# lizardfs/lizardfs

Measured on AMD Instinct MI355X. Metric: GiB/s EC encode, ec(8,2) 64MiB stripes, higher is better.
Workload: dtype u8; 1 GPU; ec(8,2) encode, 1024x64MiB synthetic stripes/GPU, device-resident; k=8, m=2, stripe_bytes=67108864, stripes_per_gpu=1024, parallelism=independent stripe batches x1

## Files before the change

lizardfs_amd/csrc/crc_fold.h:

```cpp
#pragma once
#include <hip/hip_runtime.h>

#include <cstdint>

#include "crc_fold_consts.h"

__device__ __forceinline__ uint32_t crc_advance(uint32_t crc, uint32_t len2,
                                                const uint32_t *mats) {
	int i = 0;
	while (len2) {
		if (len2 & 1) {
			const uint32_t *M = mats + i * 32;
			uint32_t r = 0, v = crc;
#pragma unroll
			for (int j = 0; j < 32; ++j) {
				r ^= (v & 1) ? M[j] : 0u;
				v >>= 1;
			}
			crc = r;
		}
		len2 >>= 1;
		++i;
	}
	return crc;
}

template <uint64_t K>
__device__ __forceinline__ void clmul_acc(uint32_t a0, uint32_t a1,
                                          uint32_t &r0, uint32_t &r1,
                                          uint32_t &r2, uint32_t &r3) {
#pragma unroll
	for (int s = 0; s < 64; ++s) {
		if ((K >> s) & 1) {
			const int t = s & 31;
			uint32_t w0 = t ? (a0 << t) : a0;
			uint32_t w1 = t ? ((a1 << t) | (a0 >> (32 - t))) : a1;
			uint32_t w2 = t ? (a1 >> (32 - t)) : 0u;
			if (s < 32) {
				r0 ^= w0;
				r1 ^= w1;
				if (t) r2 ^= w2;
			} else {
				r1 ^= w0;
				r2 ^= w1;
				if (t) r3 ^= w2;
			}
		}
	}
}

template <uint64_t KL, uint64_t KH>
__device__ __forceinline__ void crc_fold16(uint32_t (&acc)[4], uint32_t d0,
                                           uint32_t d1, uint32_t d2,
                                           uint32_t d3) {
	uint32_t r0 = d0, r1 = d1, r2 = d2, r3 = d3;
	clmul_acc<KL>(acc[0], acc[1], r0, r1, r2, r3);
	clmul_acc<KH>(acc[2], acc[3], r0, r1, r2, r3);
	acc[0] = r0;
	acc[1] = r1;
	acc[2] = r2;
	acc[3] = r3;
}

template <int NACC>
__device__ __forceinline__ void crc_fold_step(uint32_t (&acc)[4],
                                              const uint4 &d) {
	static_assert(NACC == 1 || NACC == 2 || NACC == 4, "NACC in {1,2,4}");
	if constexpr (NACC == 1)
		crc_fold16<kCrcFoldKL1, kCrcFoldKH1>(acc, d.x, d.y, d.z, d.w);
	else if constexpr (NACC == 2)
		crc_fold16<kCrcFoldKL2, kCrcFoldKH2>(acc, d.x, d.y, d.z, d.w);
	else
		crc_fold16<kCrcFoldKL4, kCrcFoldKH4>(acc, d.x, d.y, d.z, d.w);
}

__device__ __forceinline__ uint32_t crc_reduce16(const uint32_t (&acc)[4],
                                                 const uint32_t *T0) {
	uint32_t s = 0;
#pragma unroll
	for (int w = 0; w < 4; ++w) {
		uint32_t v = acc[w];
#pragma unroll
		for (int b = 0; b < 4; ++b)
			s = (s >> 8) ^ T0[(s ^ (v >> (8 * b))) & 0xFFu];
	}
	return s;
}

template <bool AL16, bool NT = false>
__device__ __forceinline__ uint4 crc_ld16(const uint8_t *p) {
	if constexpr (AL16 && NT) {
		typedef unsigned int u32x4 __attribute__((ext_vector_type(4)));
		u32x4 v = __builtin_nontemporal_load((const u32x4 *)p);
		return make_uint4(v.x, v.y, v.z, v.w);
	} else if constexpr (AL16) {
		return *(const uint4 *)p;
	} else {
		const uint32_t *u = (const uint32_t *)p;
		return make_uint4(u[0], u[1], u[2], u[3]);
	}
}

template <int C, int NACC, bool AL16 = true, bool NT = false,
          bool PF = false, int BVO = 0>
__device__ uint32_t crc_block_wave_fold(const uint8_t *__restrict__ block,
                                        uint32_t block_len, uint32_t seed,
                                        const uint32_t *T0,
                                        const uint32_t *mats, int lane) {
	constexpr int BV = BVO ? BVO : (C >= 4 ? 4 : 8);
	static_assert(BV % NACC == 0, "burst must cover whole interleave groups");
	const uint32_t span = block_len / C;
	const uint32_t seg = span >> 6;
	const uint8_t *base = block + (uint32_t)lane * seg;
	uint32_t acc[C][NACC][4];
	uint4 w[C][BV];
	auto ldburst = [&](uint4 (&buf)[C][BV], uint32_t i) {
#pragma unroll
		for (int c = 0; c < C; ++c)
#pragma unroll
			for (int q = 0; q < BV; ++q)
				buf[c][q] = crc_ld16<AL16, NT>(base + c * span + i + q * 16);
	};
	auto foldburst = [&](uint4 (&buf)[C][BV]) {
#pragma unroll
		for (int q = 0; q < BV; ++q)
#pragma unroll
			for (int c = 0; c < C; ++c)
				crc_fold_step<NACC>(acc[c][q % NACC], buf[c][q]);
	};
	ldburst(w, 0);
#pragma unroll
	for (int c = 0; c < C; ++c) {
		const uint32_t raw0 =
		    ((c == 0 && lane == 0) ? seed : 0u) ^ 0xFFFFFFFFu;
#pragma unroll
		for (int a = 0; a < NACC; ++a) {
			acc[c][a][0] = w[c][a].x ^ (a == 0 ? raw0 : 0u);
			acc[c][a][1] = w[c][a].y;
			acc[c][a][2] = w[c][a].z;
			acc[c][a][3] = w[c][a].w;
		}
#pragma unroll
		for (int q = NACC; q < BV; ++q)
			crc_fold_step<NACC>(acc[c][q % NACC], w[c][q]);
	}
	if (PF) {
		uint4 w2[C][BV];
		uint32_t i = 16 * BV;
		if (i < seg) ldburst(w2, i);
		for (; i < seg; i += 2 * 16 * BV) {
			if (i + 16 * BV < seg) ldburst(w, i + 16 * BV);
			foldburst(w2);
			if (i + 16 * BV < seg) {
				if (i + 2 * 16 * BV < seg) ldburst(w2, i + 2 * 16 * BV);
				foldburst(w);
			}
		}
	} else {
		for (uint32_t i = 16 * BV; i < seg; i += 16 * BV) {
			ldburst(w, i);
			foldburst(w);
		}
	}
	uint32_t crc[C];
#pragma unroll
	for (int c = 0; c < C; ++c) {
		uint32_t r[4] = {acc[c][0][0], acc[c][0][1], acc[c][0][2],
		                 acc[c][0][3]};
#pragma unroll
		for (int a = 1; a < NACC; ++a)
			crc_fold16<kCrcFoldKL1, kCrcFoldKH1>(
			    r, acc[c][a][0], acc[c][a][1], acc[c][a][2], acc[c][a][3]);
		crc[c] = crc_reduce16(r, T0) ^ 0xFFFFFFFFu;
	}
	uint32_t len = seg;
#pragma unroll
	for (int s = 0; s < 6; ++s) {
		uint32_t olen = __shfl_down(len, 1 << s, 64);
#pragma unroll
		for (int c = 0; c < C; ++c) {
			uint32_t o = __shfl_down(crc[c], 1 << s, 64);
			crc[c] = crc_advance(crc[c], olen, mats) ^ o;
		}
		len += olen;
	}
	uint32_t a = crc[0];
#pragma unroll
	for (int c = 1; c < C; ++c) a = crc_advance(a, span, mats) ^ crc[c];
	return a;
}
```

lizardfs_amd/csrc/crc_fold_consts.h:

```cpp
#pragma once
#include <cstdint>
constexpr uint64_t kCrcFoldKL1 = 0x420840204040300ull;
constexpr uint64_t kCrcFoldKH1 = 0x181820000810001ull;
constexpr uint64_t kCrcFoldKL2 = 0xa800004400013000ull;
constexpr uint64_t kCrcFoldKH2 = 0x20040700010021ull;
constexpr uint64_t kCrcFoldKL4 = 0x418000200010010aull;
constexpr uint64_t kCrcFoldKH4 = 0x80002200021c80ull;
```

lizardfs_amd/csrc/ec_kernel.h:

```cpp
#pragma once
#include <hip/hip_runtime.h>
#include <cstdint>

constexpr int kThreads = 256;
constexpr uint32_t kChunkBytes = kThreads * 16;

__device__ __forceinline__ uint32_t lut16(uint32_t t0, uint32_t t1,
                                          uint32_t t2, uint32_t t3,
                                          uint32_t nib) {
	uint32_t s3 = nib & 0x07070707u;
	uint32_t lo = __builtin_amdgcn_perm(t1, t0, s3);
	uint32_t hi = __builtin_amdgcn_perm(t3, t2, s3);
	uint32_t msel = 0x03020100u | ((nib >> 1) & 0x04040404u);
	return __builtin_amdgcn_perm(hi, lo, msel);
}

__device__ __forceinline__ uint32_t gf_macc(uint32_t acc, uint32_t w,
                                            const uint4 &L, const uint4 &H) {
	uint32_t nl = w & 0x0f0f0f0fu;
	uint32_t nh = (w >> 4) & 0x0f0f0f0fu;
	return acc ^ lut16(L.x, L.y, L.z, L.w, nl) ^ lut16(H.x, H.y, H.z, H.w, nh);
}

template <int D, int CH>
__device__ __forceinline__ void gf_macc_all(uint4 (&acc)[D][CH], int c,
                                            const uint4 &w, const uint4 (&L)[D],
                                            const uint4 (&H)[D]) {
#pragma unroll
	for (int d = 0; d < D; ++d) {
		acc[d][c].x = gf_macc(acc[d][c].x, w.x, L[d], H[d]);
		acc[d][c].y = gf_macc(acc[d][c].y, w.y, L[d], H[d]);
		acc[d][c].z = gf_macc(acc[d][c].z, w.z, L[d], H[d]);
		acc[d][c].w = gf_macc(acc[d][c].w, w.w, L[d], H[d]);
	}
}

__device__ __forceinline__ uint32_t gf_macc_q(uint32_t acc, const uint4 &T,
                                              uint32_t f0, uint32_t f1,
                                              uint32_t f2, uint32_t f3) {
	uint32_t p0 = __builtin_amdgcn_perm(T.x, T.x, f0);
	uint32_t p1 = __builtin_amdgcn_perm(T.y, T.y, f1);
	uint32_t p2 = __builtin_amdgcn_perm(T.z, T.z, f2);
	uint32_t p3 = __builtin_amdgcn_perm(T.w, T.w, f3);
	return acc ^ p0 ^ p1 ^ p2 ^ p3;
}

template <int D, int CH>
__device__ __forceinline__ void gf_macc_all_q(uint4 (&acc)[D][CH], int c,
                                              const uint4 &w,
                                              const uint4 (&T)[D]) {
	constexpr uint32_t M = 0x03030303u;
	uint32_t f[4][4];
	const uint32_t ws[4] = {w.x, w.y, w.z, w.w};
#pragma unroll
	for (int q = 0; q < 4; ++q) {
		f[q][0] = ws[q] & M;
		f[q][1] = (ws[q] >> 2) & M;
		f[q][2] = (ws[q] >> 4) & M;
		f[q][3] = (ws[q] >> 6) & M;
	}
#pragma unroll
	for (int d = 0; d < D; ++d) {
		acc[d][c].x = gf_macc_q(acc[d][c].x, T[d], f[0][0], f[0][1], f[0][2], f[0][3]);
		acc[d][c].y = gf_macc_q(acc[d][c].y, T[d], f[1][0], f[1][1], f[1][2], f[1][3]);
		acc[d][c].z = gf_macc_q(acc[d][c].z, T[d], f[2][0], f[2][1], f[2][2], f[2][3]);
		acc[d][c].w = gf_macc_q(acc[d][c].w, T[d], f[3][0], f[3][1], f[3][2], f[3][3]);
	}
}

__device__ __forceinline__ uint32_t gf_macc_mr(uint32_t acc, const uint4 &T,
                                               uint32_t t6, uint32_t f0,
                                               uint32_t f1, uint32_t f2) {
	uint32_t p0 = __builtin_amdgcn_perm(T.y, T.x, f0);
	uint32_t p1 = __builtin_amdgcn_perm(T.w, T.z, f1);
	uint32_t p2 = __builtin_amdgcn_perm(t6, t6, f2);
	return acc ^ p0 ^ p1 ^ p2;
}

template <int D, int CH>
__device__ __forceinline__ void gf_macc_all_mr(uint4 (&acc)[D][CH], int c,
                                               const uint4 &w,
                                               const uint4 (&T)[D],
                                               const uint4 (&T6)[D]) {
	constexpr uint32_t M3 = 0x07070707u, M2 = 0x03030303u;
	uint32_t f[4][3];
	const uint32_t ws[4] = {w.x, w.y, w.z, w.w};
#pragma unroll
	for (int q = 0; q < 4; ++q) {
		f[q][0] = ws[q] & M3;
		f[q][1] = (ws[q] >> 3) & M3;
		f[q][2] = (ws[q] >> 6) & M2;
	}
#pragma unroll
	for (int d = 0; d < D; ++d) {
		acc[d][c].x = gf_macc_mr(acc[d][c].x, T[d], T6[d].x, f[0][0], f[0][1], f[0][2]);
		acc[d][c].y = gf_macc_mr(acc[d][c].y, T[d], T6[d].x, f[1][0], f[1][1], f[1][2]);
		acc[d][c].z = gf_macc_mr(acc[d][c].z, T[d], T6[d].x, f[2][0], f[2][1], f[2][2]);
		acc[d][c].w = gf_macc_mr(acc[d][c].w, T[d], T6[d].x, f[3][0], f[3][1], f[3][2]);
	}
}

__device__ __forceinline__ uint32_t xcd_remap(uint32_t b, uint32_t n) {
	uint32_t xcd = b & 7u, i = b >> 3;
	uint32_t q = n >> 3, r = n & 7u;
	return (xcd < r ? xcd * (q + 1) : r * (q + 1) + (xcd - r) * q) + i;
}

__device__ __forceinline__ uint4 ld_nt(const uint8_t *p) {
	typedef unsigned int u32x4 __attribute__((ext_vector_type(4)));
	u32x4 v = __builtin_nontemporal_load((const u32x4 *)p);
	return make_uint4(v.x, v.y, v.z, v.w);
}

template <int D, int CH, bool SWZ, bool NTST, bool NTLD = false,
          bool TPIPE = false, bool QL = false, bool MR = false>
__global__ __launch_bounds__(kThreads) void ec_encode_kernel(
    uint32_t part_len, int srcs, int dest_base,
    const uint8_t *__restrict__ gftbls_dev,
    const uint64_t *__restrict__ src_ptrs,
    const uint64_t *__restrict__ dst_ptrs,
    int dests_total, uint32_t tiles_per_part, uint32_t total_tiles) {
	static_assert(!(QL && TPIPE), "QL and TPIPE are mutually exclusive");
	static_assert(!(MR && (QL || TPIPE)), "MR excludes QL/TPIPE");
	constexpr uint32_t kTile = kChunkBytes * CH;
	extern __shared__ __attribute__((aligned(16))) uint8_t smem[];
	const uint32_t tid = threadIdx.x;

	{
		const int tw = QL ? 16 : 32;
		const uint8_t *src_tbl = gftbls_dev + (size_t)dest_base * srcs * tw;
		int nbytes = D * srcs * tw;
		for (int i = tid * 16; i < nbytes; i += kThreads * 16)
			*(uint4 *)(smem + i) = *(const uint4 *)(src_tbl + i);
	}
	__syncthreads();

	uint32_t b0 = SWZ ? xcd_remap(blockIdx.x, gridDim.x) : blockIdx.x;
	for (uint32_t tile = b0; tile < total_tiles; tile += gridDim.x) {
		uint32_t stripe = tile / tiles_per_part;
		uint32_t tin = tile - stripe * tiles_per_part;
		uint32_t base = tin * kTile + tid * 16u;
		const uint64_t *sp_tab = src_ptrs + (uint64_t)stripe * srcs;
		const uint64_t *dp_tab =
		    dst_ptrs + (uint64_t)stripe * dests_total + dest_base;

		uint4 acc[D][CH];
#pragma unroll
		for (int d = 0; d < D; ++d)
#pragma unroll
			for (int c = 0; c < CH; ++c)
				acc[d][c] = make_uint4(0, 0, 0, 0);

		if ((uint64_t)(tin + 1) * kTile <= part_len) {
			uint4 w[CH], wn[CH];
			uint4 L[TPIPE ? 2 : 1][D], H[QL ? 1 : (TPIPE ? 2 : 1)][D];
			auto tbl_read = [&](int j, uint4 (&Lb)[D], uint4 (&Hb)[D]) {
#pragma unroll
				for (int d = 0; d < D; ++d) {
					if (QL) {
						Lb[d] = *(const uint4 *)(smem +
						                         ((size_t)d * srcs + j) * 16);
					} else if (MR) {
						const uint8_t *tb =
						    smem + ((size_t)d * srcs + j) * 32;
						Lb[d] = *(const uint4 *)tb;
						Hb[d].x = *(const uint32_t *)(tb + 16);
					} else {
						const uint8_t *tb =
						    smem + ((size_t)d * srcs + j) * 32;
						Lb[d] = *(const uint4 *)tb;
						Hb[d] = *(const uint4 *)(tb + 16);
					}
				}
			};
			{
				const uint8_t *sp = (const uint8_t *)sp_tab[0];
#pragma unroll
				for (int c = 0; c < CH; ++c)
					w[c] = NTLD ? ld_nt(sp + (base + c * kChunkBytes))
					            : *(const uint4 *)(sp + (base + c * kChunkBytes));
			}
			auto step = [&](int j, uint4 (&Lc)[D], uint4 (&Hc)[D],
			                uint4 (&Ln)[D], uint4 (&Hn)[D]) {
				if (j + 1 < srcs) {
					const uint8_t *spn = (const uint8_t *)sp_tab[j + 1];
#pragma unroll
					for (int c = 0; c < CH; ++c)
						wn[c] = NTLD ? ld_nt(spn + (base + c * kChunkBytes))
						             : *(const uint4 *)(spn + (base + c * kChunkBytes));
					if (TPIPE) tbl_read(j + 1, Ln, Hn);
				}
				if (!TPIPE) tbl_read(j, Lc, Hc);
#pragma unroll
				for (int c = 0; c < CH; ++c) {
					if (QL)
						gf_macc_all_q<D, CH>(acc, c, w[c], Lc);
					else if (MR)
						gf_macc_all_mr<D, CH>(acc, c, w[c], Lc, Hc);
					else
						gf_macc_all<D, CH>(acc, c, w[c], Lc, Hc);
				}
#pragma unroll
				for (int c = 0; c < CH; ++c) w[c] = wn[c];
			};
			if (TPIPE) tbl_read(0, L[0], H[0]);
			int j = 0;
			for (; j + 1 < srcs; j += 2) {
				step(j, L[0], H[0], L[TPIPE ? 1 : 0], H[TPIPE ? 1 : 0]);
				step(j + 1, L[TPIPE ? 1 : 0], H[TPIPE ? 1 : 0], L[0], H[0]);
			}
			if (j < srcs) step(j, L[0], H[0], L[TPIPE ? 1 : 0], H[TPIPE ? 1 : 0]);
#pragma unroll
			for (int d = 0; d < D; ++d) {
				uint8_t *dp = (uint8_t *)dp_tab[d];
#pragma unroll
				for (int c = 0; c < CH; ++c) {
					uint4 *p = (uint4 *)(dp + (base + c * kChunkBytes));
					if (NTST) {
						typedef unsigned int u32x4
						    __attribute__((ext_vector_type(4)));
						u32x4 v = {acc[d][c].x, acc[d][c].y, acc[d][c].z,
						           acc[d][c].w};
						__builtin_nontemporal_store(v, (u32x4 *)p);
					} else {
						*p = acc[d][c];
					}
				}
			}
		} else {
// ... 47 lines not shown
```

lizardfs_amd/csrc/lizec_gpu.hip:

```cpp
#include <hip/hip_runtime.h>

#include <cstdint>
#include <cstdio>
#include <cstring>
#include <cstdlib>
#include <atomic>
#include <mutex>
#include <unordered_map>

#include "../../include/lizec.h"

#define LIZEC_CHECK(x)                                                   \
	do {                                                                 \
		hipError_t _e = (x);                                             \
		if (_e != hipSuccess) return LIZEC_EHIP;                         \
	} while (0)

#include "ec_kernel.h"
#include "ec_kernel_multi.h"
#include "ec_kernel_strided.h"
#include "ec_kernel_ragged.h"
#include "ec_kernel_view.h"
#include "crc_fold.h"
#include "crc_ranges.h"
// ... 52 lines not shown
		      T1[(u >> 16) & 0xff] ^ T0[u >> 24];                      \
	} while (0)
			LIZEC_CRC_WORD(w.x);
			LIZEC_CRC_WORD(w.y);
			LIZEC_CRC_WORD(w.z);
			LIZEC_CRC_WORD(w.w);
#undef LIZEC_CRC_WORD
		}
		crc ^= 0xFFFFFFFFu;

		uint32_t len = seg;
#pragma unroll
		for (int s = 0; s < 6; ++s) {
			uint32_t ocrc = __shfl_down(crc, 1 << s, 64);
			uint32_t olen = __shfl_down(len, 1 << s, 64);
			crc = crc_advance(crc, olen, mats) ^ ocrc;
			len += olen;
		}
		if (lane == 0) out[blk] = crc;
	}
}

template <int C, int BV, int SL = 16>
__device__ uint32_t crc_block_wave(const uint8_t *__restrict__ block,
                                   uint32_t block_len, uint32_t seed,
                                   const uint32_t *T, const uint32_t *mats,
                                   int lane) {
	const uint32_t span = block_len / C;
	const uint32_t seg = span >> 6;
	const uint8_t *base = block + (uint32_t)lane * seg;
	uint32_t crc[C];
#pragma unroll
	for (int c = 0; c < C; ++c)
		crc[c] = ((c == 0 && lane == 0) ? seed : 0u) ^ 0xFFFFFFFFu;
	for (uint32_t i = 0; i < seg; i += 16 * BV) {
		uint4 w[C][BV];
#pragma unroll
		for (int c = 0; c < C; ++c)
#pragma unroll
			for (int q = 0; q < BV; ++q)
				w[c][q] = *(const uint4 *)(base + c * span + i + q * 16);
#define LIZEC_CRC16(crc, v)                                              \
	do {                                                                 \
		uint32_t u0 = (crc) ^ (v).x, u1 = (v).y, u2 = (v).z, u3 = (v).w; \
		(crc) = T[15 * 256 + (u0 & 0xff)] ^                              \
		        T[14 * 256 + ((u0 >> 8) & 0xff)] ^                       \
		        T[13 * 256 + ((u0 >> 16) & 0xff)] ^                      \
		        T[12 * 256 + (u0 >> 24)] ^                               \
		        T[11 * 256 + (u1 & 0xff)] ^                              \
		        T[10 * 256 + ((u1 >> 8) & 0xff)] ^                       \
		        T[9 * 256 + ((u1 >> 16) & 0xff)] ^                       \
		        T[8 * 256 + (u1 >> 24)] ^                                \
		        T[7 * 256 + (u2 & 0xff)] ^                               \
		        T[6 * 256 + ((u2 >> 8) & 0xff)] ^                        \
		        T[5 * 256 + ((u2 >> 16) & 0xff)] ^                       \
		        T[4 * 256 + (u2 >> 24)] ^                                \
		        T[3 * 256 + (u3 & 0xff)] ^                               \
		        T[2 * 256 + ((u3 >> 8) & 0xff)] ^                        \
		        T[1 * 256 + ((u3 >> 16) & 0xff)] ^ T[u3 >> 24];          \
	} while (0)
#define LIZEC_CRC8(crc, lo, hi)                                          \
	do {                                                                 \
		uint32_t u0 = (crc) ^ (lo), u1 = (hi);                           \
		(crc) = T[7 * 256 + (u0 & 0xff)] ^                               \
		        T[6 * 256 + ((u0 >> 8) & 0xff)] ^                        \
		        T[5 * 256 + ((u0 >> 16) & 0xff)] ^                       \
		        T[4 * 256 + (u0 >> 24)] ^                                \
		        T[3 * 256 + (u1 & 0xff)] ^                               \
		        T[2 * 256 + ((u1 >> 8) & 0xff)] ^                        \
		        T[1 * 256 + ((u1 >> 16) & 0xff)] ^ T[u1 >> 24];          \
	} while (0)
#pragma unroll
		for (int q = 0; q < BV; ++q)
#pragma unroll
			for (int c = 0; c < C; ++c) {
				if (SL == 16) {
					LIZEC_CRC16(crc[c], w[c][q]);
				} else {
					LIZEC_CRC8(crc[c], w[c][q].x, w[c][q].y);
					LIZEC_CRC8(crc[c], w[c][q].z, w[c][q].w);
				}
			}
#undef LIZEC_CRC16
#undef LIZEC_CRC8
	}
#pragma unroll
	for (int c = 0; c < C; ++c) crc[c] ^= 0xFFFFFFFFu;

	uint32_t len = seg;
#pragma unroll
	for (int s = 0; s < 6; ++s) {
		uint32_t olen = __shfl_down(len, 1 << s, 64);
#pragma unroll
		for (int c = 0; c < C; ++c) {
			uint32_t o = __shfl_down(crc[c], 1 << s, 64);
			crc[c] = crc_advance(crc[c], olen, mats) ^ o;
		}
		len += olen;
	}
	uint32_t acc = crc[0];
#pragma unroll
	for (int c = 1; c < C; ++c)
		acc = crc_advance(acc, span, mats) ^ crc[c];
	return acc;
}

template <int C, int BV, int SL = 16>
__global__ __launch_bounds__(kThreads) void crc32_blocks_kernel_multi(
    const uint8_t *__restrict__ buf, uint32_t block_len, uint64_t nblocks,
    uint32_t seed, const uint32_t *__restrict__ crc_const,
    uint32_t *__restrict__ out) {
	__shared__ __attribute__((aligned(16))) uint32_t stabs[kCrcConstWords];
	for (int i = threadIdx.x; i < kCrcConstWords; i += kThreads)
		stabs[i] = crc_const[i];
	__syncthreads();
	const uint32_t *T = stabs;
	const uint32_t *mats = stabs + kCrcTabWords;
	const int wave = threadIdx.x >> 6;
	const int lane = threadIdx.x & 63;
	for (uint64_t blk = (uint64_t)blockIdx.x * 4 + wave; blk < nblocks;
	     blk += (uint64_t)gridDim.x * 4) {
		uint32_t crc = crc_block_wave<C, BV, SL>(buf + blk * block_len,
		                                         block_len, seed, T, mats,
		                                         lane);
		if (lane == 0) out[blk] = crc;
	}
}


constexpr int kCrcFoldLdsWords = 256 + kCrcMatCount * 32;

template <int C, int NACC, bool AL16 = true, bool NT = false,
          bool PF = false, int BVO = 0>
__global__ __launch_bounds__(kThreads) void crc32_blocks_kernel_fold(
    const uint8_t *__restrict__ buf, uint32_t block_len, uint64_t nblocks,
    uint32_t seed, const uint32_t *__restrict__ crc_const,
    uint32_t *__restrict__ out) {
	__shared__ __attribute__((aligned(16))) uint32_t stabs[kCrcFoldLdsWords];
	for (int i = threadIdx.x; i < 256; i += kThreads)
		stabs[i] = crc_const[i];
	for (int i = threadIdx.x; i < kCrcMatCount * 32; i += kThreads)
		stabs[256 + i] = crc_const[kCrcTabWords + i];
	__syncthreads();
	const int wave = threadIdx.x >> 6;
	const int lane = threadIdx.x & 63;
	for (uint64_t blk = (uint64_t)blockIdx.x * 4 + wave; blk < nblocks;
	     blk += (uint64_t)gridDim.x * 4) {
		uint32_t crc = crc_block_wave_fold<C, NACC, AL16, NT, PF, BVO>(
		    buf + blk * block_len, block_len, seed, stabs, stabs + 256, lane);
		if (lane == 0) out[blk] = crc;
	}
}

template <bool WRITE>
__global__ __launch_bounds__(kThreads) void scrub_chunks_kernel(
    const uint64_t *__restrict__ chunk_dptrs,
    const uint32_t *__restrict__ data_offs,
    const uint32_t *__restrict__ crc_offs,
    const uint32_t *__restrict__ block_counts, uint32_t nchunks,
    uint32_t max_blocks, uint32_t block_stride, uint32_t crc_stride,
    const uint32_t *__restrict__ crc_const, int32_t *__restrict__ status) {
	__shared__ __attribute__((aligned(16))) uint32_t stabs[kCrcFoldLdsWords];
	for (int i = threadIdx.x; i < 256; i += kThreads)
		stabs[i] = crc_const[i];
	for (int i = threadIdx.x; i < kCrcMatCount * 32; i += kThreads)
		stabs[256 + i] = crc_const[kCrcTabWords + i];
	__syncthreads();
	const uint32_t *T0 = stabs;
	const uint32_t *mats = stabs + 256;
	const int wave = threadIdx.x >> 6;
	const int lane = threadIdx.x & 63;
	const uint64_t total = (uint64_t)nchunks * max_blocks;
	for (uint64_t flat = (uint64_t)blockIdx.x * 4 + wave; flat < total;
	     flat += (uint64_t)gridDim.x * 4) {
		uint32_t c = (uint32_t)(flat / max_blocks);
		uint32_t b = (uint32_t)(flat - (uint64_t)c * max_blocks);
		if (b >= block_counts[c]) continue;
		const uint8_t *img = (const uint8_t *)chunk_dptrs[c];
		const uint8_t *blockp = img + data_offs[c] + b * block_stride;
		uint32_t crc =
		    (((uintptr_t)blockp & 15) == 0)
		        ? crc_block_wave_fold<1, 1, true>(blockp, 65536u, 0u, T0,
		                                          mats, lane)
		        : crc_block_wave_fold<1, 1, false>(blockp, 65536u, 0u, T0,
		                                           mats, lane);
		if (lane == 0) {
			uint8_t *p = (uint8_t *)img + crc_offs[c] + crc_stride * b;
			if (WRITE) {
				p[0] = (uint8_t)(crc >> 24);
				p[1] = (uint8_t)(crc >> 16);
				p[2] = (uint8_t)(crc >> 8);
				p[3] = (uint8_t)crc;
			} else {
				uint32_t stored = ((uint32_t)p[0] << 24) |
				                  ((uint32_t)p[1] << 16) |
				                  ((uint32_t)p[2] << 8) | p[3];
				if (stored != crc) atomicMin(&status[c], (int32_t)b);
			}
		}
	}
}


struct lizec_stream_ctx {
	uint8_t *d_gftbls = nullptr;
	uint64_t *d_ptrs = nullptr;
	size_t ptrs_cap = 0;
	uint8_t *h_staging = nullptr;
	size_t h_cap = 0;
	hipEvent_t uploaded = nullptr;
	bool ev_recorded = false;
	uint8_t *d_mtbls = nullptr;
	size_t mtbls_cap = 0;
	uint32_t *d_mindex = nullptr;
	size_t mindex_cap = 0;
	uint8_t *h_mstaging = nullptr;
	size_t h_mcap = 0;
	uint8_t *d_ragged = nullptr;
	uint8_t *h_ragged = nullptr;
	size_t ragged_cap = 0;
};

struct lizec_engine {
	int device;
	hipStream_t stream;
	uint32_t *d_crc_const;
	std::mutex mu;
	std::unordered_map<void *, lizec_stream_ctx> ctxs;
	std::atomic<int> crc_shape{-1};
};

static void ctx_free(lizec_stream_ctx &c) {
	(void)hipFree(c.d_gftbls);
	(void)hipFree(c.d_ptrs);
	(void)hipHostFree(c.h_staging);
	(void)hipFree(c.d_mtbls);
	(void)hipFree(c.d_mindex);
	(void)hipHostFree(c.h_mstaging);
	(void)hipFree(c.d_ragged);
	(void)hipHostFree(c.h_ragged);
	if (c.uploaded) (void)hipEventDestroy(c.uploaded);
	c = lizec_stream_ctx();
}

static int ctx_acquire(lizec_engine *e, hipStream_t s, size_t ptrs,
                       size_t staging, lizec_stream_ctx **out) {
	lizec_stream_ctx *cp;
	{
		std::lock_guard<std::mutex> lk(e->mu);
		cp = &e->ctxs[(void *)s];
	}
	lizec_stream_ctx &c = *cp;
	if (!c.uploaded) {
		if (hipEventCreateWithFlags(&c.uploaded, hipEventDisableTiming) !=
		    hipSuccess)
			return LIZEC_EHIP;
	}
	if (c.ev_recorded) {
		LIZEC_CHECK(hipEventSynchronize(c.uploaded));
		c.ev_recorded = false;
	}
	if (!c.d_gftbls)
		LIZEC_CHECK(hipMalloc(&c.d_gftbls, (size_t)kECTblBytes * 32 * 32));
	if (c.ptrs_cap < ptrs) {
		size_t cap = c.ptrs_cap ? c.ptrs_cap : (1 << 16);
		while (cap < ptrs) cap *= 2;
		(void)hipFree(c.d_ptrs);
		c.d_ptrs = nullptr;
		c.ptrs_cap = 0;
		LIZEC_CHECK(hipMalloc(&c.d_ptrs, cap * sizeof(uint64_t)));
		c.ptrs_cap = cap;
	}
	size_t want = staging + (size_t)kECTblBytes * 32 * 32;
	if (c.h_cap < want) {
		size_t cap = c.h_cap ? c.h_cap : (1 << 20);
		while (cap < want) cap *= 2;
		(void)hipHostFree(c.h_staging);
		c.h_staging = nullptr;
		c.h_cap = 0;
		LIZEC_CHECK(hipHostMalloc(&c.h_staging, cap));
		c.h_cap = cap;
	}
	*out = &c;
	return LIZEC_OK;
}

static int ctx_acquire_multi(lizec_engine *e, hipStream_t s, size_t ptrs,
                             size_t staging, size_t tbl_bytes, size_t stripes,
                             lizec_stream_ctx **out) {
	int r = ctx_acquire(e, s, ptrs, staging, out);
	if (r != LIZEC_OK) return r;
	lizec_stream_ctx &c = **out;
	if (c.mtbls_cap < tbl_bytes) {
		size_t cap = c.mtbls_cap ? c.mtbls_cap : (1 << 16);
		while (cap < tbl_bytes) cap *= 2;
		(void)hipFree(c.d_mtbls);
		c.d_mtbls = nullptr;
		c.mtbls_cap = 0;
		LIZEC_CHECK(hipMalloc(&c.d_mtbls, cap));
		c.mtbls_cap = cap;
	}
	if (c.mindex_cap < stripes) {
		size_t cap = c.mindex_cap ? c.mindex_cap : (1 << 14);
		while (cap < stripes) cap *= 2;
		(void)hipFree(c.d_mindex);
		c.d_mindex = nullptr;
		c.mindex_cap = 0;
		LIZEC_CHECK(hipMalloc(&c.d_mindex, cap * sizeof(uint32_t)));
		c.mindex_cap = cap;
	}
	size_t want = tbl_bytes + stripes * sizeof(uint32_t);
	if (c.h_mcap < want) {
		size_t cap = c.h_mcap ? c.h_mcap : (1 << 17);
		while (cap < want) cap *= 2;
		(void)hipHostFree(c.h_mstaging);
		c.h_mstaging = nullptr;
		c.h_mcap = 0;
		LIZEC_CHECK(hipHostMalloc(&c.h_mstaging, cap));
		c.h_mcap = cap;
	}
	return LIZEC_OK;
}

static int ctx_acquire_ragged(lizec_engine *e, hipStream_t s, size_t ptrs,
                              size_t staging, size_t bytes,
                              lizec_stream_ctx **out) {
	int r = ctx_acquire(e, s, ptrs, staging, out);
	if (r != LIZEC_OK) return r;
	lizec_stream_ctx &c = **out;
	if (c.ragged_cap < bytes) {
		size_t cap = c.ragged_cap ? c.ragged_cap : (1 << 17);
		while (cap < bytes) cap *= 2;
		(void)hipFree(c.d_ragged);
		(void)hipHostFree(c.h_ragged);
		c.d_ragged = c.h_ragged = nullptr;
		c.ragged_cap = 0;
		LIZEC_CHECK(hipMalloc(&c.d_ragged, cap));
		LIZEC_CHECK(hipHostMalloc(&c.h_ragged, cap));
// ... 706 lines not shown
	                           hipMemcpyHostToDevice, s));
	LIZEC_CHECK(hipMemcpyAsync(c->d_mindex, istage, (size_t)num_stripes * 4,
	                           hipMemcpyHostToDevice, s));
	LIZEC_CHECK(hipMemcpyAsync(d_src, pstage, (nsrc + ndst) * 8,
	                           hipMemcpyHostToDevice, s));
	LIZEC_CHECK(hipEventRecord(c->uploaded, s));
	c->ev_recorded = true;

	return run_batch_multi(part_len, srcs, dests, c->d_mtbls, c->d_mindex,
	                       d_src, d_dst, (uint32_t)num_stripes, s);
}

extern "C" int lizec_ec_plan_create_multi(lizec_engine *e, uint64_t part_len,
                                          int srcs, int dests,
                                          const uint8_t *gftbls, int ntables,
                                          const uint32_t *tbl_index,
                                          const uint64_t *src_dptrs,
                                          const uint64_t *dst_dptrs,
                                          int num_stripes, lizec_plan **out) {
	*out = nullptr;
	if (!e) return LIZEC_EINVAL;
	int r = check_multi_args(part_len, srcs, dests, gftbls, ntables,
	                         tbl_index, src_dptrs, dst_dptrs, num_stripes);
	if (r != LIZEC_OK) return r;
	LIZEC_CHECK(hipSetDevice(e->device));
	size_t nsrc = (size_t)num_stripes * srcs;
	size_t ndst = (size_t)num_stripes * dests;
	size_t ntbl = (size_t)ntables * srcs * dests;
	size_t tbl_bytes = ntbl * kECTblBytes;
	uint8_t *packed = (uint8_t *)malloc(tbl_bytes);
	if (!packed) return LIZEC_ENOMEM;
	for (size_t i = 0; i < ntbl; ++i)
		pack_mixed_radix(gftbls + i * 32, packed + i * kECTblBytes);
	lizec_plan *p = new lizec_plan();
	p->e = e;
	p->part_len = part_len;
	p->srcs = srcs;
	p->dests = dests;
	p->num_stripes = num_stripes;
	if (hipMalloc(&p->d_tbls, tbl_bytes) != hipSuccess ||
	    hipMalloc(&p->d_src, nsrc * 8) != hipSuccess ||
	    hipMalloc(&p->d_dst, ndst * 8) != hipSuccess ||
	    hipMalloc(&p->d_index, (size_t)num_stripes * 4) != hipSuccess) {
		free(packed);
		lizec_ec_plan_destroy(p);
		return LIZEC_ENOMEM;
	}
	bool ok = hipMemcpy(p->d_tbls, packed, tbl_bytes,
	                    hipMemcpyHostToDevice) == hipSuccess &&
	          hipMemcpy(p->d_index, tbl_index, (size_t)num_stripes * 4,
	                    hipMemcpyHostToDevice) == hipSuccess &&
	          hipMemcpy(p->d_src, src_dptrs, nsrc * 8,
	                    hipMemcpyHostToDevice) == hipSuccess &&
	          hipMemcpy(p->d_dst, dst_dptrs, ndst * 8,
	                    hipMemcpyHostToDevice) == hipSuccess;
	free(packed);
	if (!ok) {
		lizec_ec_plan_destroy(p);
		return LIZEC_EHIP;
	}
	*out = p;
	return LIZEC_OK;
}

extern "C" int lizec_ec_plan_create(lizec_engine *e, uint64_t part_len,
                                    int srcs, int dests,
                                    const uint8_t *gftbls,
                                    const uint64_t *src_dptrs,
                                    const uint64_t *dst_dptrs,
                                    int num_stripes, lizec_plan **out) {
	*out = nullptr;
	if (!e) return LIZEC_EINVAL;
	int r = check_batch_args(part_len, srcs, dests, num_stripes);
	if (r != LIZEC_OK) return r;
	size_t nsrc = (size_t)num_stripes * srcs;
	size_t ndst = (size_t)num_stripes * dests;
	r = check_part_addrs(src_dptrs, nsrc, dst_dptrs, ndst);
	if (r != LIZEC_OK) return r;
	LIZEC_CHECK(hipSetDevice(e->device));
	lizec_plan *p = new lizec_plan();
	p->e = e;
	p->part_len = part_len;
	p->srcs = srcs;
	p->dests = dests;
	p->num_stripes = num_stripes;
	if (hipMalloc(&p->d_tbls, (size_t)kECTblBytes * srcs * dests) != hipSuccess ||
	    hipMalloc(&p->d_src, nsrc * 8) != hipSuccess ||
	    hipMalloc(&p->d_dst, ndst * 8) != hipSuccess) {
		lizec_ec_plan_destroy(p);
		return LIZEC_ENOMEM;
	}
	uint8_t packed[kECTblBytes * 32 * 32];
	for (int i = 0; i < srcs * dests; ++i)
		pack_mixed_radix(gftbls + (size_t)i * 32, packed + (size_t)i * kECTblBytes);
	if (hipMemcpy(p->d_tbls, packed, (size_t)kECTblBytes * srcs * dests,
	              hipMemcpyHostToDevice) != hipSuccess ||
	    hipMemcpy(p->d_src, src_dptrs, nsrc * 8,
	              hipMemcpyHostToDevice) != hipSuccess ||
	    hipMemcpy(p->d_dst, dst_dptrs, ndst * 8,
	              hipMemcpyHostToDevice) != hipSuccess) {
		lizec_ec_plan_destroy(p);
		return LIZEC_EHIP;
	}
	*out = p;
	return LIZEC_OK;
}

extern "C" int lizec_ec_plan_run(lizec_plan *p, void *stream) {
	if (!p) return LIZEC_EINVAL;
	hipStream_t s = stream ? (hipStream_t)stream : p->e->stream;
	LIZEC_CHECK(hipSetDevice(p->e->device));
	if (p->d_index)
		return run_batch_multi(p->part_len, p->srcs, p->dests, p->d_tbls,
		                       p->d_index, p->d_src, p->d_dst,
		                       (uint32_t)p->num_stripes, s);
	return run_batch(p->part_len, p->srcs, p->dests, p->d_tbls, p->d_src,
	                 p->d_dst, (uint32_t)p->num_stripes, s);
}

extern "C" void lizec_ec_plan_destroy(lizec_plan *p) {
	if (!p) return;
	(void)hipFree(p->d_tbls);
	(void)hipFree(p->d_src);
	(void)hipFree(p->d_dst);
	(void)hipFree(p->d_index);
	delete p;
}

extern "C" int lizec_crc32_batch(lizec_engine *e, const void *dev_buf,
                                 uint32_t block_len, uint64_t nblocks,
                                 uint32_t seed, uint32_t *dev_crcs_out,
                                 void *stream) {
	if (!e || !dev_buf || !dev_crcs_out || nblocks < 1) return LIZEC_EINVAL;
	if (block_len == 0 || (block_len & 1023)) return LIZEC_EINVAL;
	if (block_len >= (2u << kCrcMatCount)) return LIZEC_EINVAL;
	if ((uintptr_t)dev_buf & 3) return LIZEC_EINVAL;
	hipStream_t s = stream ? (hipStream_t)stream : e->stream;
	LIZEC_CHECK(hipSetDevice(e->device));
	uint64_t groups = (nblocks + 3) / 4;
	uint32_t grid = (uint32_t)(groups < 131072 ? groups : 131072);
	const char *ch = getenv("LIZEC_CRC_CHAINS");
	const char *sl = getenv("LIZEC_CRC_SLICE");
	const char *im = getenv("LIZEC_CRC_IMPL");
	const char *fn = getenv("LIZEC_CRC_FOLD_NACC");
	const char *nt = getenv("LIZEC_CRC_NT");
	const char *pf = getenv("LIZEC_CRC_PF");
	int chains = ch ? atoi(ch) : 1;
	int slice = sl ? atoi(sl) : 8;
	bool fold = !(im && strcmp(im, "table") == 0);
	int nacc = fn ? atoi(fn) : 1;
	bool ntld = nt && atoi(nt) != 0;
	bool pfld = pf && atoi(pf) != 0;
	bool al16 = (((uintptr_t)dev_buf | block_len) & 15) == 0;
	if (!al16 && (!fold || block_len % (64 * 16 * 8) != 0)) {
		hipLaunchKernelGGL(HIP_KERNEL_NAME(crc32_blocks_kernel<false>),
		                   dim3(grid), dim3(kThreads), 0, s,
		                   (const uint8_t *)dev_buf, block_len, nblocks,
		                   seed, e->d_crc_const, dev_crcs_out);
		LIZEC_CHECK(hipGetLastError());
		return LIZEC_OK;
	}
	if (!al16 && !(chains == 2 && block_len % (2 * 64 * 16 * 8) == 0))
		chains = 1;
	if (fold && block_len % ((uint32_t)chains * 64 * 16 * 8) == 0 &&
	    (chains == 1 || chains == 2)) {
		const uint8_t *b = (const uint8_t *)dev_buf;
#define LIZEC_LAUNCH_FOLD(C, N, A, NT)                                       \
	hipLaunchKernelGGL(HIP_KERNEL_NAME(crc32_blocks_kernel_fold<C, N, A, NT>), \
	                   dim3(grid), dim3(kThreads), 0, s, b, block_len,       \
	                   nblocks, seed, e->d_crc_const, dev_crcs_out)
		if (!al16) {
			if (chains == 2) LIZEC_LAUNCH_FOLD(2, 2, false, false);
			else LIZEC_LAUNCH_FOLD(1, 1, false, false);
		} else if (chains == 2) {
			if (nacc == 1) LIZEC_LAUNCH_FOLD(2, 1, true, false);
			else LIZEC_LAUNCH_FOLD(2, 2, true, false);
		} else if (pfld) {
			const char *bv = getenv("LIZEC_CRC_BV");
			if (bv && atoi(bv) == 4)
				hipLaunchKernelGGL(HIP_KERNEL_NAME(crc32_blocks_kernel_fold<1, 1, true, false, true, 4>),
				                   dim3(grid), dim3(kThreads), 0, s, b,
				                   block_len, nblocks, seed, e->d_crc_const,
				                   dev_crcs_out);
			else
				hipLaunchKernelGGL(HIP_KERNEL_NAME(crc32_blocks_kernel_fold<1, 1, true, false, true>),
				                   dim3(grid), dim3(kThreads), 0, s, b,
				                   block_len, nblocks, seed, e->d_crc_const,
				                   dev_crcs_out);
		} else if (ntld) {
			if (nacc == 1) LIZEC_LAUNCH_FOLD(1, 1, true, true);
			else if (nacc == 4) LIZEC_LAUNCH_FOLD(1, 4, true, true);
			else LIZEC_LAUNCH_FOLD(1, 2, true, true);
		} else {
			const char *bv = getenv("LIZEC_CRC_BV");
			const char *at = getenv("LIZEC_CRC_AUTOTUNE");
			bool tune = !(at && atoi(at) == 0);
			if (bv && atoi(bv) == 4 && nacc == 1) {
				hipLaunchKernelGGL(HIP_KERNEL_NAME(crc32_blocks_kernel_fold<1, 1, true, false, false, 4>),
				                   dim3(grid), dim3(kThreads), 0, s, b,
				                   block_len, nblocks, seed, e->d_crc_const,
				                   dev_crcs_out);
			} else if (nacc == 4) {
				if (bv && atoi(bv) == 4)
					hipLaunchKernelGGL(HIP_KERNEL_NAME(crc32_blocks_kernel_fold<1, 4, true, false, false, 4>),
					                   dim3(grid), dim3(kThreads), 0, s, b,
					                   block_len, nblocks, seed,
					                   e->d_crc_const, dev_crcs_out);
				else
					LIZEC_LAUNCH_FOLD(1, 4, true, false);
			} else if (nacc == 2) {
				if (bv && atoi(bv) == 4)
					hipLaunchKernelGGL(HIP_KERNEL_NAME(crc32_blocks_kernel_fold<1, 2, true, false, false, 4>),
					                   dim3(grid), dim3(kThreads), 0, s, b,
					                   block_len, nblocks, seed,
					                   e->d_crc_const, dev_crcs_out);
				else
					LIZEC_LAUNCH_FOLD(1, 2, true, false);
			} else {
				int shape = e->crc_shape.load(std::memory_order_relaxed);
				if (shape < 0 && tune && nblocks >= 4096) {
					hipEvent_t ev[3];
					int made = 0;
					for (; made < 3; ++made)
						if (hipEventCreate(&ev[made]) != hipSuccess) break;
					if (made == 3) {
						(void)hipEventRecord(ev[0], s);
						LIZEC_LAUNCH_FOLD(1, 1, true, false);
						(void)hipEventRecord(ev[1], s);
						hipLaunchKernelGGL(HIP_KERNEL_NAME(crc32_blocks_kernel_fold<1, 1, true, false, true>),
						                   dim3(grid), dim3(kThreads), 0, s,
						                   b, block_len, nblocks, seed,
						                   e->d_crc_const, dev_crcs_out);
						(void)hipEventRecord(ev[2], s);
						if (hipEventSynchronize(ev[2]) == hipSuccess) {
							float t0 = 0.f, t1 = 0.f;
							(void)hipEventElapsedTime(&t0, ev[0], ev[1]);
							(void)hipEventElapsedTime(&t1, ev[1], ev[2]);
							shape = (t1 > 0.f && t1 < t0) ? 1 : 0;
							e->crc_shape.store(shape,
							                   std::memory_order_relaxed);
						}
					} else {
						LIZEC_LAUNCH_FOLD(1, 1, true, false);
					}
					for (int i = 0; i < made; ++i)
						(void)hipEventDestroy(ev[i]);
					LIZEC_CHECK(hipGetLastError());
					return LIZEC_OK;
				}
				if (shape == 1)
					hipLaunchKernelGGL(HIP_KERNEL_NAME(crc32_blocks_kernel_fold<1, 1, true, false, true>),
					                   dim3(grid), dim3(kThreads), 0, s, b,
					                   block_len, nblocks, seed,
					                   e->d_crc_const, dev_crcs_out);
				else
					LIZEC_LAUNCH_FOLD(1, 1, true, false);
			}
		}
#undef LIZEC_LAUNCH_FOLD
		LIZEC_CHECK(hipGetLastError());
		return LIZEC_OK;
	}
	if (block_len % 32768 == 0 && chains >= 4)
		hipLaunchKernelGGL(HIP_KERNEL_NAME(crc32_blocks_kernel_multi<4, 8>),
		                   dim3(grid), dim3(kThreads), 0, s,
		                   (const uint8_t *)dev_buf, block_len, nblocks,
		                   seed, e->d_crc_const, dev_crcs_out);
	else if (block_len % 16384 == 0 && slice == 8)
		hipLaunchKernelGGL(HIP_KERNEL_NAME(crc32_blocks_kernel_multi<2, 8, 8>),
		                   dim3(grid), dim3(kThreads), 0, s,
		                   (const uint8_t *)dev_buf, block_len, nblocks,
		                   seed, e->d_crc_const, dev_crcs_out);
	else if (block_len % 16384 == 0)
		hipLaunchKernelGGL(HIP_KERNEL_NAME(crc32_blocks_kernel_multi<2, 8>),
		                   dim3(grid), dim3(kThreads), 0, s,
		                   (const uint8_t *)dev_buf, block_len, nblocks,
		                   seed, e->d_crc_const, dev_crcs_out);
	else
		hipLaunchKernelGGL(HIP_KERNEL_NAME(crc32_blocks_kernel<true>),
		                   dim3(grid), dim3(kThreads), 0, s,
		                   (const uint8_t *)dev_buf, block_len, nblocks,
		                   seed, e->d_crc_const, dev_crcs_out);
	LIZEC_CHECK(hipGetLastError());
	return LIZEC_OK;
}


static_assert(kCrcRangesMats <= kCrcMatCount, "matrix bank too short");
static_assert(sizeof(lizec_write_op) == 40, "lizec_write_op has padding");

constexpr uint32_t kCrcRangesMaxN = 1u << 24;
constexpr uint32_t kCrcRangesMaxGrid = 16384;

static int launch_crc_ranges(lizec_engine *e, const uint64_t *d_addrs,
                             const uint32_t *d_lens, uint32_t n, uint32_t seed,
                             uint32_t *d_out, uint32_t *d_nz, hipStream_t s) {
	uint32_t groups = (n + 3) / 4;
	uint32_t grid = groups < kCrcRangesMaxGrid ? groups : kCrcRangesMaxGrid;
	if (d_nz)
		hipLaunchKernelGGL(HIP_KERNEL_NAME(crc32_ranges_kernel<true>),
		                   dim3(grid), dim3(kCrcRangesThreads), 0, s, d_addrs,
		                   d_lens, n, seed, e->d_crc_const,
		                   e->d_crc_const + kCrcTabWords, d_out, d_nz);
	else
		hipLaunchKernelGGL(HIP_KERNEL_NAME(crc32_ranges_kernel<false>),
		                   dim3(grid), dim3(kCrcRangesThreads), 0, s, d_addrs,
// ... 486 lines not shown
```

Before: 4645 GiB/s.

## Add wide-window sparse CRC fold kernel and use three-input XOR in GF kernels

Result: no change. 4667 GiB/s, median of 6 (+0.5%).

```diff
diff --git a/lizardfs_amd/csrc/crc_fold.h b/lizardfs_amd/csrc/crc_fold.h
--- a/lizardfs_amd/csrc/crc_fold.h
+++ b/lizardfs_amd/csrc/crc_fold.h
@@ -2,6 +2,7 @@
 #include <hip/hip_runtime.h>
 
 #include <cstdint>
+#include <type_traits>
 
 #include "crc_fold_consts.h"
 
@@ -189,3 +190,144 @@
 	for (int c = 1; c < C; ++c) a = crc_advance(a, span, mats) ^ crc[c];
 	return a;
 }
+
+
+
+__device__ __forceinline__ uint32_t crc_xor3(uint32_t a, uint32_t b,
+                                             uint32_t c) {
+#if defined(__HIP_DEVICE_COMPILE__)
+	return __builtin_amdgcn_bitop3_b32(a, b, c, 0x96);
+#else
+	return a ^ b ^ c;
+#endif
+}
+
+template <int I, int N, class F>
+__device__ __forceinline__ void crc_static_for(F &&f) {
+	if constexpr (I < N) {
+		f(std::integral_constant<int, I>{});
+		crc_static_for<I + 1, N>(f);
+	}
+}
+
+constexpr bool crc_wide_compiled(int nbits) {
+	return nbits == 384 || nbits == 1024 || nbits == 2048;
+}
+
+constexpr int crc_wide_kbit(int nbits, int b) {
+	return nbits == 384 ? kCrcWideK384[b]
+	     : nbits == 1024 ? kCrcWideK1024[b] : kCrcWideK2048[b];
+}
+
+constexpr bool crc_wide_touches(int nbits, int b, int j) {
+	const int p = crc_wide_kbit(nbits, b);
+	const int k = j - (p >> 5);
+	return k >= 0 && k < ((p & 31) ? 5 : 4);
+}
+
+template <int NBITS, int B, int J>
+__device__ __forceinline__ uint32_t crc_wide_term(const uint32_t (&L)[4]) {
+	constexpr int p = crc_wide_kbit(NBITS, B);
+	constexpr int t = p & 31, k = J - (p >> 5);
+	if constexpr (t == 0)
+		return L[k];
+	else if constexpr (k == 0)
+		return L[0] << t;
+	else if constexpr (k == 4)
+		return L[3] >> (32 - t);
+	else
+		return (L[k] << t) | (L[k - 1] >> (32 - t));
+}
+
+template <int NBITS>
+__device__ __forceinline__ void crc_wide_mul_acc(const uint32_t (&L)[4],
+                                                 uint32_t (&W)[NBITS / 32]) {
+	static_assert(crc_wide_kbit(NBITS, 3) < NBITS - 127,
+	              "the product must stay inside the window");
+	crc_static_for<0, NBITS / 32>([&](auto J) {
+		constexpr int j = decltype(J)::value;
+		uint32_t acc = W[j], pend = 0;
+		bool have = false;
+		crc_static_for<0, 4>([&](auto B) {
+			constexpr int b = decltype(B)::value;
+			if constexpr (crc_wide_touches(NBITS, b, j)) {
+				const uint32_t t = crc_wide_term<NBITS, b, j>(L);
+				if (have)
+					acc = crc_xor3(acc, pend, t);
+				else
+					pend = t;
+				have = !have;
+			}
+		});
+		if (have) acc ^= pend;
+		W[j] = acc;
+	});
+}
+
+template <int NBITS, bool AL16 = true>
+__device__ __forceinline__ uint32_t crc_block_wave_fold_wide(
+    const uint8_t *__restrict__ block, uint32_t block_len, uint32_t seed,
+    const uint32_t *T0, const uint32_t *mats, int lane) {
+	static_assert(crc_wide_compiled(NBITS), "no constant for this window");
+	constexpr int BV = 8;
+	constexpr int NW = NBITS / 32;
+	constexpr int NV = NBITS / 128;
+	constexpr int NFILL = (NV + BV - 1) / BV;
+	constexpr int UNR = NW % 32 == 0 ? (NW > 32 ? NW / 32 : 1) : 3;
+	const uint32_t seg = block_len >> 6;
+	const uint8_t *base = block + (uint32_t)lane * seg;
+	uint32_t W[NW];
+	uint4 d[BV];
+	auto ldburst = [&](uint32_t i) {
+#pragma unroll
+		for (int q = 0; q < BV; ++q) d[q] = crc_ld16<AL16>(base + i + q * 16);
+	};
+	auto step = [&](const uint4 &v) {
+		const uint32_t L[4] = {W[0], W[1], W[2], W[3]};
+#pragma unroll
+		for (int i = 0; i + 4 < NW; ++i) W[i] = W[i + 4];
+		W[NW - 4] = v.x;
+		W[NW - 3] = v.y;
+		W[NW - 2] = v.z;
+		W[NW - 1] = v.w;
+		crc_wide_mul_acc<NBITS>(L, W);
+	};
+#pragma unroll
+	for (int g = 0; g < NFILL; ++g) {
+		ldburst(g * 16 * BV);
+#pragma unroll
+		for (int q = 0; q < BV; ++q) {
+			if (g * BV + q < NV) {
+				W[4 * (g * BV + q) + 0] = d[q].x;
+				W[4 * (g * BV + q) + 1] = d[q].y;
+				W[4 * (g * BV + q) + 2] = d[q].z;
+				W[4 * (g * BV + q) + 3] = d[q].w;
+				if (g == 0 && q == 0)
+					W[0] ^= (lane == 0 ? seed : 0u) ^ 0xFFFFFFFFu;
+			} else {
+				step(d[q]);
+			}
+		}
+	}
+#pragma unroll UNR
+	for (uint32_t i = NFILL * 16 * BV; i < seg; i += 16 * BV) {
+		ldburst(i);
+#pragma unroll
+		for (int q = 0; q < BV; ++q) step(d[q]);
+	}
+	uint32_t r[4] = {W[0], W[1], W[2], W[3]};
+#pragma unroll
+	for (int a = 1; a < NV; ++a)
+		crc_fold16<kCrcFoldKL1, kCrcFoldKH1>(r, W[4 * a], W[4 * a + 1],
+		                                     W[4 * a + 2], W[4 * a + 3]);
+	uint32_t crc = crc_reduce16(r, T0) ^ 0xFFFFFFFFu;
+	uint32_t len = seg;
+#pragma unroll
+	for (int s = 0; s < 6; ++s) {
+		uint32_t olen = __shfl_down(len, 1 << s, 64);
+		uint32_t o = __shfl_down(crc, 1 << s, 64);
+		crc = crc_advance(crc, olen, mats) ^ o;
+		len += olen;
+	}
+	return crc;
+}
diff --git a/lizardfs_amd/csrc/crc_fold_consts.h b/lizardfs_amd/csrc/crc_fold_consts.h
--- a/lizardfs_amd/csrc/crc_fold_consts.h
+++ b/lizardfs_amd/csrc/crc_fold_consts.h
@@ -6,3 +6,6 @@
 constexpr uint64_t kCrcFoldKH2 = 0x20040700010021ull;
 constexpr uint64_t kCrcFoldKL4 = 0x418000200010010aull;
 constexpr uint64_t kCrcFoldKH4 = 0x80002200021c80ull;
+constexpr int kCrcWideK384[4] = {17, 55, 83, 172};
+constexpr int kCrcWideK1024[4] = {88, 192, 562, 873};
+constexpr int kCrcWideK2048[4] = {640, 776, 1152, 1561};
diff --git a/lizardfs_amd/csrc/ec_kernel.h b/lizardfs_amd/csrc/ec_kernel.h
--- a/lizardfs_amd/csrc/ec_kernel.h
+++ b/lizardfs_amd/csrc/ec_kernel.h
@@ -4,6 +4,15 @@
 
 constexpr int kThreads = 256;
 constexpr uint32_t kChunkBytes = kThreads * 16;
+
+__device__ __forceinline__ uint32_t gf_xor3(uint32_t a, uint32_t b,
+                                            uint32_t c) {
+#if defined(__HIP_DEVICE_COMPILE__)
+	return __builtin_amdgcn_bitop3_b32(a, b, c, 0x96);
+#else
+	return a ^ b ^ c;
+#endif
+}
 
 __device__ __forceinline__ uint32_t lut16(uint32_t t0, uint32_t t1,
                                           uint32_t t2, uint32_t t3,
@@ -19,7 +28,8 @@
                                             const uint4 &L, const uint4 &H) {
 	uint32_t nl = w & 0x0f0f0f0fu;
 	uint32_t nh = (w >> 4) & 0x0f0f0f0fu;
-	return acc ^ lut16(L.x, L.y, L.z, L.w, nl) ^ lut16(H.x, H.y, H.z, H.w, nh);
+	return gf_xor3(acc, lut16(L.x, L.y, L.z, L.w, nl),
+	               lut16(H.x, H.y, H.z, H.w, nh));
 }
 
 template <int D, int CH>
@@ -42,7 +52,7 @@
 	uint32_t p1 = __builtin_amdgcn_perm(T.y, T.y, f1);
 	uint32_t p2 = __builtin_amdgcn_perm(T.z, T.z, f2);
 	uint32_t p3 = __builtin_amdgcn_perm(T.w, T.w, f3);
-	return acc ^ p0 ^ p1 ^ p2 ^ p3;
+	return gf_xor3(gf_xor3(acc, p0, p1), p2, p3);
 }
 
 template <int D, int CH>
@@ -74,7 +84,7 @@
 	uint32_t p0 = __builtin_amdgcn_perm(T.y, T.x, f0);
 	uint32_t p1 = __builtin_amdgcn_perm(T.w, T.z, f1);
 	uint32_t p2 = __builtin_amdgcn_perm(t6, t6, f2);
-	return acc ^ p0 ^ p1 ^ p2;
+	return gf_xor3(acc, p0, p1) ^ p2;
 }
 
 template <int D, int CH>
diff --git a/lizardfs_amd/csrc/lizec_gpu.hip b/lizardfs_amd/csrc/lizec_gpu.hip
--- a/lizardfs_amd/csrc/lizec_gpu.hip
+++ b/lizardfs_amd/csrc/lizec_gpu.hip
@@ -228,6 +228,38 @@
 	}
 }
 
+constexpr int kCrcWideBits = 384;
+
+template <int NBITS, bool AL16 = true>
+__global__ __launch_bounds__(kThreads) void crc32_blocks_kernel_wide(
+    const uint8_t *__restrict__ buf, uint32_t block_len, uint64_t nblocks,
+    uint32_t seed, const uint32_t *__restrict__ crc_const,
+    uint32_t *__restrict__ out) {
+	__shared__ __attribute__((aligned(16))) uint32_t stabs[kCrcFoldLdsWords];
+	for (int i = threadIdx.x; i < 256; i += kThreads)
+		stabs[i] = crc_const[i];
+	for (int i = threadIdx.x; i < kCrcMatCount * 32; i += kThreads)
+		stabs[256 + i] = crc_const[kCrcTabWords + i];
+	__syncthreads();
+	const int wave = threadIdx.x >> 6;
+	const int lane = threadIdx.x & 63;
+	for (uint64_t blk = (uint64_t)blockIdx.x * 4 + wave; blk < nblocks;
+	     blk += (uint64_t)gridDim.x * 4) {
+		uint32_t crc = crc_block_wave_fold_wide<NBITS, AL16>(
+		    buf + blk * block_len, block_len, seed, stabs, stabs + 256, lane);
+		if (lane == 0) out[blk] = crc;
+	}
+}
+
+template <bool AL16>
+__device__ __noinline__ uint32_t scrub_block_crc(const uint8_t *block,
+                                                 const uint32_t *T0,
+                                                 const uint32_t *mats,
+                                                 int lane) {
+	return crc_block_wave_fold_wide<kCrcWideBits, AL16>(block, 65536u, 0u, T0,
+	                                                    mats, lane);
+}
+
 template <bool WRITE>
 __global__ __launch_bounds__(kThreads) void scrub_chunks_kernel(
     const uint64_t *__restrict__ chunk_dptrs,
@@ -256,10 +288,8 @@
 		const uint8_t *blockp = img + data_offs[c] + b * block_stride;
 		uint32_t crc =
 		    (((uintptr_t)blockp & 15) == 0)
-		        ? crc_block_wave_fold<1, 1, true>(blockp, 65536u, 0u, T0,
-		                                          mats, lane)
-		        : crc_block_wave_fold<1, 1, false>(blockp, 65536u, 0u, T0,
-		                                           mats, lane);
+		        ? scrub_block_crc<true>(blockp, T0, mats, lane)
+		        : scrub_block_crc<false>(blockp, T0, mats, lane);
 		if (lane == 0) {
 			uint8_t *p = (uint8_t *)img + crc_offs[c] + crc_stride * b;
 			if (WRITE) {
@@ -1272,6 +1302,32 @@
 	bool ntld = nt && atoi(nt) != 0;
 	bool pfld = pf && atoi(pf) != 0;
 	bool al16 = (((uintptr_t)dev_buf | block_len) & 15) == 0;
+	if (!ch && !fn && !nt && !pf && !getenv("LIZEC_CRC_BV") &&
+	    (!im || strcmp(im, "wide") == 0) && block_len % (64 * 16 * 8) == 0) {
+		const char *wb = getenv("LIZEC_CRC_WIDE_BITS");
+		int bits = wb ? atoi(wb) : kCrcWideBits;
+		if (!crc_wide_compiled(bits)) bits = kCrcWideBits;
+		if (block_len / 64 >= (uint32_t)bits / 8) {
+#define LIZEC_LAUNCH_WIDE(N, A)                                              \
+	hipLaunchKernelGGL(HIP_KERNEL_NAME(crc32_blocks_kernel_wide<N, A>),      \
+	                   dim3(grid), dim3(kThreads), 0, s,                     \
+	                   (const uint8_t *)dev_buf, block_len, nblocks, seed,   \
+	                   e->d_crc_const, dev_crcs_out)
+			if (bits == 384) {
+				if (al16) LIZEC_LAUNCH_WIDE(384, true);
+				else LIZEC_LAUNCH_WIDE(384, false);
+			} else if (bits == 2048) {
+				if (al16) LIZEC_LAUNCH_WIDE(2048, true);
+				else LIZEC_LAUNCH_WIDE(2048, false);
+			} else {
+				if (al16) LIZEC_LAUNCH_WIDE(1024, true);
+				else LIZEC_LAUNCH_WIDE(1024, false);
+			}
+#undef LIZEC_LAUNCH_WIDE
+			LIZEC_CHECK(hipGetLastError());
+			return LIZEC_OK;
+		}
+	}
 	if (!al16 && (!fold || block_len % (64 * 16 * 8) != 0)) {
 		hipLaunchKernelGGL(HIP_KERNEL_NAME(crc32_blocks_kernel<false>),
 		                   dim3(grid), dim3(kThreads), 0, s,
```
